# ryansynk/fastmax-experiments

Hardware: AMD Instinct MI355X
Metric: fastmax attn tokens/sec + achieved HBM GB/s at N=4096 d=64, 1/8 GPU (higher is better)
Workload: dtype f32; 1 GPU; fastmax p=1 masked fwd, (B,H,N,D)=(16,32,4096,64) per GPU, q,k,v~N(0,1) seed=rank, f32 I/O, fp32 accumulate; B_per_gpu=16, H=32, N=4096, D=64, global_batch=16, parallelism=dp1 (batch sharded, no data-path collective)

## Files before the change

fastmax_experiments_amd/csrc/fastmax_api.hip:

```cpp
#include "fastmax_common.h"

#include <climits>
#include <cstdlib>
#include <cstring>

using namespace fastmax;

namespace {
bool use_bf16_kernel(const fastmax_problem& p) {
    return mfma_bf16_supported(p) && tune_get(TUNE_BF16_KERNEL) != 0;
}
int validate(const fastmax_problem* p) {
    if (!p) return FASTMAX_E_NULL;
    if (p->p != 1 && p->p != 2) return FASTMAX_E_BAD_P;
    if (p->B <= 0 || p->H <= 0 || p->Nq <= 0 || p->Nk <= 0 || p->D <= 0 || p->D > FASTMAX_MAX_D)
        return FASTMAX_E_BAD_SHAPE;
    if (p->causal && p->Nq != p->Nk) return FASTMAX_E_BAD_SHAPE;
    if ((int64_t)p->B * p->H > 65535) return FASTMAX_E_BAD_SHAPE;
    if (p->in_dtype < 0 || p->in_dtype > 2 || p->out_dtype < 0 || p->out_dtype > 2) return FASTMAX_E_BAD_DTYPE;
    return FASTMAX_OK;
}
Strides3 st(const int64_t* s) { return Strides3{s[0], s[1], s[2]}; }

int select(const fastmax_problem& p) {
// ... 92 lines not shown
    if (p.path != FASTMAX_PATH_QUADRATIC_MFMA && has(lay, LAY_O)) {
        if (unmasked_lin_bwd_supported(p)) return FASTMAX_BWD_UNMASKED_LIN;
        if (lin_bwd_supported(p) && p.in_dtype == p.out_dtype) return FASTMAX_BWD_LIN;
        if (scan_bwd_supported(p)) return FASTMAX_BWD_SCAN;
    }
    return quad32_bwd_supported(p) ? FASTMAX_BWD_QUAD32 : FASTMAX_BWD_QUAD_MFMA;
}

int normalize_check(bool have_ptrs, int B, int H, int rep, int N, int D, const void* workspace, size_t workspace_bytes, size_t need,
                    int dtype = FASTMAX_F32) {
    if (!have_ptrs) return FASTMAX_E_NULL;
    if (B <= 0 || H <= 0 || rep <= 0 || N <= 0 || D <= 0 || D > FASTMAX_MAX_D) return FASTMAX_E_BAD_SHAPE;
    if (dtype < 0 || dtype > FASTMAX_F16) return FASTMAX_E_BAD_DTYPE;
    if (!workspace || workspace_bytes < need) return FASTMAX_E_WORKSPACE;
    return FASTMAX_OK;
}
}

namespace fastmax {
static bool mfma_variant_ok(int v) {
#ifdef FASTMAX_ABLATIONS
    if (v == 201 || (v >= 204 && v <= 209)) return true;
#endif
    return v == 200;
}
namespace {
struct TuneEntry { const char* name; const char* env; int value; };
TuneEntry g_tune[TUNE_COUNT] = {
    {"mfma_variant", "FASTMAX_MFMA_VARIANT", 200},
    {"bf16_kernel", "FASTMAX_BF16_KERNEL", 1},
    {"gemm_sched", "FASTMAX_GEMM_SCHED", 0},
    {"gemm_group_m", "FASTMAX_GEMM_GROUP_M", 16},
    {"gemm_xcd", "FASTMAX_GEMM_XCD", 1},
};
bool g_tune_loaded = false;
void tune_load() {
    if (g_tune_loaded) return;
    for (int i = 0; i < TUNE_COUNT; ++i) {
        const char* e = getenv(g_tune[i].env);
        if (!e) continue;
        if (i == TUNE_BF16_KERNEL) g_tune[i].value = e[0] == 'g' ? 0 : 1;
        else g_tune[i].value = atoi(e);
        if (i == TUNE_MFMA_VARIANT && !mfma_variant_ok(g_tune[i].value)) g_tune[i].value = 200;
    }
    g_tune_loaded = true;
}
}
int tune_get(int key) {
    tune_load();
    return g_tune[key].value;
}
int tune_set(const char* name, int value) {
    tune_load();
    for (int i = 0; i < TUNE_COUNT; ++i)
        if (!strcmp(name, g_tune[i].name)) {
            if (i == TUNE_MFMA_VARIANT && !mfma_variant_ok(value)) return FASTMAX_E_BAD_SHAPE;
            g_tune[i].value = value;
            return FASTMAX_OK;
        }
    return FASTMAX_E_BAD_SHAPE;
}
int tune_get_by_name(const char* name) {
    tune_load();
    for (int i = 0; i < TUNE_COUNT; ++i)
        if (!strcmp(name, g_tune[i].name)) return g_tune[i].value;
    return INT_MIN;
// ... 313 lines not shown
```

fastmax_experiments_amd/csrc/fastmax_common.h:

```cpp
#pragma once
#include <hip/hip_runtime.h>
#include <hip/hip_bf16.h>
#include <hip/hip_fp16.h>
#include <stdint.h>

#include "../../include/fastmax_hip.h"

namespace fastmax {

struct bf16_t { uint16_t bits; };
struct f16_t { _Float16 v; };

__device__ __forceinline__ float to_float(float x) { return x; }
__device__ __forceinline__ float to_float(bf16_t x) { return __uint_as_float(((uint32_t)x.bits) << 16); }
__device__ __forceinline__ float to_float(f16_t x) { return (float)x.v; }

__device__ __forceinline__ uint16_t f32_to_bf16_bits(float f) {
    __hip_bfloat16 h = __float2bfloat16(f);
    return *reinterpret_cast<uint16_t*>(&h);
}
template <typename T> __device__ __forceinline__ T from_float(float f);
template <> __device__ __forceinline__ float from_float<float>(float f) { return f; }
template <> __device__ __forceinline__ bf16_t from_float<bf16_t>(float f) { return bf16_t{f32_to_bf16_bits(f)}; }
template <> __device__ __forceinline__ f16_t from_float<f16_t>(float f) { return f16_t{(_Float16)f}; }
// ... 55 lines not shown
    int *nstar_q = nullptr, *nstar_k = nullptr;
};
struct FwdArgs {
    fastmax_problem prob;
    const void *q, *k, *v;
    Strides3 qs, ks, vs;
    void* o;
    float* g;
    void* workspace;
    size_t workspace_bytes;
    hipStream_t stream;
    const LinearmaxStats* stats = nullptr;
};
struct BwdArgs {
    fastmax_problem prob;
    const void *q, *k, *v, *o, *grad_o;
    const float* g;
    Strides3 qs, ks, vs, gos;
    void *dq, *dk, *dv;
    void* workspace;
    size_t workspace_bytes;
    hipStream_t stream;
    const float* fwd_states = nullptr;
    const float *qscale = nullptr, *kscale = nullptr;
    int fuse_prologue = 0;
    const int* k_nstar = nullptr;
    const int* q_nstar = nullptr;
};

int launch_fwd_quadratic(const FwdArgs& a);
int launch_fwd_recurrent_p1(const FwdArgs& a);
int launch_fwd_mfma_p1(const FwdArgs& a);
bool mfma_p1_supported(const fastmax_problem& p);
enum TuneKey { TUNE_MFMA_VARIANT = 0, TUNE_BF16_KERNEL = 1, TUNE_GEMM_SCHED = 2, TUNE_GEMM_GROUP_M = 3, TUNE_GEMM_XCD = 4, TUNE_COUNT };
int tune_get(int key);
int tune_set(const char* name, int value);
int tune_get_by_name(const char* name);
int launch_fwd_mfma_gen(const FwdArgs& a, const float* qscale, const float* kscale);
int launch_fwd_mfma_bf16(const FwdArgs& a, const float* qscale, const float* kscale);
bool mfma_bf16_supported(const fastmax_problem& p);
bool mfma_gen_supported(const fastmax_problem& p, bool norm);
int launch_normalize_cast(const void* x, Strides3 xs, int dtype, void* y, const float* inv_norm, int B, int H, int N, int D,
                          hipStream_t stream, const unsigned int* partials = nullptr, int npart = 0, float* inv_out = nullptr, int rep = 1);
int launch_normalize_partial_max(const void* x, Strides3 xs, int dtype, unsigned int* partials, int B, int H, int N, int D,
                                 hipStream_t stream);
size_t normalize_backward_workspace(int B, int H, int N);
size_t normalize_backward_workspace_grouped(int B, int G, int rep, int N);
int normalize_block_tokens(int rep);
int launch_normalize_backward(const void* x, Strides3 xs, int dtype, const void* gy, const float* inv_norm, void* gx, int B, int H,
                              int N, int D, void* ws, hipStream_t stream, int rep = 1);
int launch_normalize_stats(const void* x, Strides3 xs, int dtype, float* inv_norm, int B, int H, int N, int D,
                           void* workspace, hipStream_t stream);
int launch_normalize_stats2(const void* x0, Strides3 s0, const void* x1, Strides3 s1, int dtype, float* inv0, float* inv1, int B, int H,
                            int N, int D, void* ws, hipStream_t stream, int* nstar0 = nullptr, int* nstar1 = nullptr);
struct SplitPlan { int nseg, cps; };
SplitPlan split_plan(const fastmax_problem& p);
size_t split_workspace_bytes(const fastmax_problem& p, int dp);
int launch_split_states(const FwdArgs& a, const SplitPlan& plan, int dp, const float* kscale);
int linearmax_stats_and_states(const FwdArgs& a, const SplitPlan& plan, int dp);
bool unmasked_lin_supported(const fastmax_problem& p);
size_t unmasked_lin_workspace(const fastmax_problem& p);
int launch_fwd_unmasked_p1(const FwdArgs& a);
int launch_bwd_unmasked_p1(const BwdArgs& a);
size_t unmasked_lin_bwd_workspace(const fastmax_problem& p);
bool unmasked_lin_bwd_supported(const fastmax_problem& p);
int launch_bwd_prep_c(const BwdArgs& a, float* cbuf);
int launch_normalize_fixadd(const void* x, Strides3 xs, int dtype, const float* inv_norm, const float* part_dot,
// ... 29 lines not shown
```

fastmax_experiments_amd/csrc/fastmax_mfma32_common.h:

```cpp
#pragma once
#include "fastmax_mfma_common.h"

namespace fastmax {

typedef float f32x16 __attribute__((ext_vector_type(16)));

__device__ __forceinline__ f32x16 mfma32(const bf16x8 a, const bf16x8 b, f32x16 c) {
    return __builtin_amdgcn_mfma_f32_32x32x16_bf16(a, b, c, 0, 0, 0);
}
__device__ __forceinline__ f32x16 mfma32_c1(const bf16x8 a, const bf16x8 b) {
    f32x16 d;
    asm("s_nop 1\n\tv_mfma_f32_32x32x16_bf16 %0, %1, %2, 1.0\n\ts_nop 11" : "=&v"(d) : "v"(a), "v"(b));
    return d;
}
template <int NA, int NB>
__device__ __forceinline__ f32x16 mfma32_parts_c1(const Frag<NA>& a, const Frag<NB>& b) {
    f32x16 c = mfma32_c1(a.p[0], b.p[0]);
    if constexpr (NA == 2) c = mfma32(a.p[1], b.p[0], c);
    if constexpr (NB == 2) c = mfma32(a.p[0], b.p[1], c);
    return c;
}
template <int NA, int NB>
__device__ __forceinline__ f32x16 mfma32_parts(const Frag<NA>& a, const Frag<NB>& b, f32x16 c) {
    c = mfma32(a.p[0], b.p[0], c);
    if constexpr (NA == 2) c = mfma32(a.p[1], b.p[0], c);
    if constexpr (NB == 2) c = mfma32(a.p[0], b.p[1], c);
    return c;
}

__device__ __forceinline__ void mfma32_acc(f32x16& acc, const bf16x8 a, const bf16x8 b) {
    asm("s_nop 1\n\tv_mfma_f32_32x32x16_bf16 %0, %1, %2, %0" : "+a"(acc) : "v"(a), "v"(b));
}
template <int NA, int NB>
__device__ __forceinline__ void mfma32_parts_acc(f32x16& acc, const Frag<NA>& a, const Frag<NB>& b) {
    mfma32_acc(acc, a.p[0], b.p[0]);
    if constexpr (NA == 2) mfma32_acc(acc, a.p[1], b.p[0]);
    if constexpr (NB == 2) mfma32_acc(acc, a.p[0], b.p[1]);
}
// ... 118 lines not shown
```

fastmax_experiments_amd/csrc/fastmax_quad32_bwd.hip:

```cpp
#include "fastmax_mfma32_common.h"

#include <cmath>
#include <cstdlib>
#include <type_traits>

namespace fastmax {

struct Quad32BwdParams {
    const void *q, *k, *v, *gt;
    const float* cw;
    Strides3 qs, ks, vs;
    void *dq, *dk, *dv;
    int H, BH, Nq, Nk, D, causal, grad_dtype, nblk;
    float a;
};

__device__ __forceinline__ void quad32_block(int L, int nblk, int BH, int& bh, int& blk) {
    if ((BH & 7) == 0) {
        const int x = L & 7, m = L >> 3;
        bh = x + 8 * (m / nblk);
        blk = m % nblk;
    } else {
        bh = L / nblk;
        blk = L % nblk;
    }
}

template <int NPP> __device__ __forceinline__ void pack_tile(const float (&x)[16], Frag<NPP> (&f)[2]) {
#pragma unroll
    for (int s = 0; s < 2; ++s) {
        const f32x4 x0 = {x[8 * s], x[8 * s + 1], x[8 * s + 2], x[8 * s + 3]};
        const f32x4 x1 = {x[8 * s + 4], x[8 * s + 5], x[8 * s + 6], x[8 * s + 7]};
        if constexpr (NPP == 2) {
            bf16x4 h0, l0, h1, l1;
            split4(x0, h0, l0);
            split4(x1, h1, l1);
            f[s].p[0] = cat4(h0, h1);
            f[s].p[1] = cat4(l0, l1);
        } else {
            f[s].p[0] = cat4(to_bf16x4(x0), to_bf16x4(x1));
        }
    }
}

template <int NP, bool UNIT>
__device__ __forceinline__ f32x16 s_chain_head(const Frag<NP>& a, const Frag<NP>& b, const f32x16& cinit) {
    if constexpr (UNIT) return mfma32_parts_c1<NP, NP>(a, b);
    else return mfma32_parts<NP, NP>(a, b, cinit);
}

template <int DP, int P, typename TIN, int NW, int MB, bool UNIT>
__global__ __launch_bounds__(64 * NW, MB) void bwd32_dq_kernel(Quad32BwdParams prm) {
    constexpr int NP = InTraits<TIN>::NP, EPL = InTraits<TIN>::EPL, NPP = NP;
    constexpr int NT = 64 * NW, QT = 32 * NW;
    constexpr bool DUAL = DP == 128 && NP == 1;
    constexpr int SWR = DUAL ? 1 : 3, SWT = DUAL ? 2 : 3;
    constexpr int IMG = img_bytes<DP, SWR>(), IMGT = DUAL ? img_bytes<DP, SWT>() : 0;
    constexpr int KTO = 2 * NP * IMG, STAGE = 2 * NP * IMG + NP * IMGT;
    constexpr int COLS = DP / EPL, RPP = NT / COLS, NPASS = 64 / RPP;
    static_assert(RPP <= 64 && NPASS >= 1, "staging map");
    constexpr int KS = DP / 16, DT = DP / 32;
    constexpr bool ACC_A = DP == 128 && MB == 1;
    extern __shared__ __attribute__((aligned(16))) char smem[];
    const int tid = threadIdx.x, lane = tid & 63;
    const int w = __builtin_amdgcn_readfirstlane(tid >> 6);
    const int l31 = lane & 31, h = lane >> 5;
    int bh, qt;
    quad32_block(blockIdx.x, prm.nblk, prm.BH, bh, qt);
    const bool causal = prm.causal != 0;
    if (causal) qt = prm.nblk - 1 - qt;
    const int b = bh / prm.H, hh = bh % prm.H;
    const int D = prm.D, Nq = prm.Nq, Nk = prm.Nk;
    const int i0 = qt * QT, qw0 = i0 + 32 * w, myq = qw0 + l31;
    const TIN* qb = reinterpret_cast<const TIN*>(prm.q) + (int64_t)b * prm.qs.sb + (int64_t)hh * prm.qs.sh;
    const TIN* kb = reinterpret_cast<const TIN*>(prm.k) + (int64_t)b * prm.ks.sb + (int64_t)hh * prm.ks.sh;
    const TIN* vb = reinterpret_cast<const TIN*>(prm.v) + (int64_t)b * prm.vs.sb + (int64_t)hh * prm.vs.sh;
    const TIN* gb = reinterpret_cast<const TIN*>(prm.gt) + (int64_t)bh * Nq * D;
    const int srow = tid / COLS, scol = tid % COLS;

    Frag<NP> qf[KS], gf[KS];
#pragma unroll
    for (int ks = 0; ks < KS; ++ks) {
        if constexpr (P == 2) {
            if constexpr (UNIT) qf[ks] = load_q_frag_scaled<TIN>(qb, prm.qs.sn, myq, Nq, 16 * ks + 8 * h, D, prm.a);
            else qf[ks] = load_q_frag<TIN>(qb, prm.qs.sn, myq, Nq, 16 * ks + 8 * h, D);
        }
        gf[ks] = load_q_frag<TIN>(gb, D, myq, Nq, 16 * ks + 8 * h, D);
    }
    const int qc = myq < Nq ? myq : Nq - 1;
    const float ncw = -prm.cw[(int64_t)bh * Nq + qc];
    f32x16 ucinit, scinit;
#pragma unroll
    for (int i = 0; i < 16; ++i) { ucinit[i] = ncw; scinit[i] = 1.0f / prm.a; }
    const int klim = causal ? min(myq, Nk - 1) : Nk - 1;

    u32x4 rk[NPASS], rv[NPASS];
    const TileKernelLoader<TIN, NPASS, RPP> kload(kb, prm.ks.sn, Nk, D, srow, scol), vload(vb, prm.vs.sn, Nk, D, srow, scol);
    auto request = [&](int kt) __attribute__((always_inline)) {
        kload.load(kt, rk);
        vload.load(kt, rv);
    };
// ... 87 lines not shown
        advance(kt);
        tile(kt, kt & 1, std::true_type{});
        __syncthreads();
    }
    for (; kt < nkt; ++kt) {
        advance(kt);
        __syncthreads();
    }
    if constexpr (ACC_A) {
#pragma unroll
        for (int mt = 0; mt < DT; ++mt) acc_fence(acc[mt]);
    }
    const float oscale = (P == 2 && !UNIT) ? prm.a * prm.a : prm.a;
    store_tile32_t<DT>(smem + w * 4096, acc, oscale, lane, prm.dq, prm.grad_dtype, (int64_t)bh * Nq, qw0, Nq, D);
}

template <int DP, int P, typename TIN, int NW, bool UNIT>
__global__ __launch_bounds__(64 * NW, (DP == 64 && InTraits<TIN>::NP == 1 && NW == 4) ? 2 : 1) void bwd32_dkv_kernel(Quad32BwdParams prm) {
    constexpr int NP = InTraits<TIN>::NP, EPL = InTraits<TIN>::EPL, NPP = NP;
    constexpr int NT = 64 * NW, KT = 32 * NW;
    constexpr bool DUAL = DP == 128 && NP == 1;
    constexpr int SWR = DUAL ? 1 : 3, SWT = DUAL ? 2 : 3;
    constexpr int IMG = img_bytes<DP, SWR>(), IMGT = DUAL ? img_bytes<DP, SWT>() : 0;
    constexpr int TRO = 2 * NP * IMG, CWO = TRO + 2 * NP * IMGT, STAGE = CWO + 256;
    constexpr int COLS = DP / EPL, RPP = NT / COLS, NPASS = 64 / RPP;
    static_assert(RPP <= 64 && NPASS >= 1, "staging map");
    constexpr int KS = DP / 16, DT = DP / 32;
    constexpr bool ACC_A = DP == 128 && NW == 4;
    extern __shared__ __attribute__((aligned(16))) char smem[];
    const int tid = threadIdx.x, lane = tid & 63;
    const int w = __builtin_amdgcn_readfirstlane(tid >> 6);
    const int l31 = lane & 31, h = lane >> 5;
    int bh, kb_;
    quad32_block(blockIdx.x, prm.nblk, prm.BH, bh, kb_);
    const bool causal = prm.causal != 0;
    const int b = bh / prm.H, hh = bh % prm.H;
    const int D = prm.D, Nq = prm.Nq, Nk = prm.Nk;
    const int j0 = kb_ * KT, jw0 = j0 + 32 * w, myk = jw0 + l31;
    const TIN* qb = reinterpret_cast<const TIN*>(prm.q) + (int64_t)b * prm.qs.sb + (int64_t)hh * prm.qs.sh;
    const TIN* kb = reinterpret_cast<const TIN*>(prm.k) + (int64_t)b * prm.ks.sb + (int64_t)hh * prm.ks.sh;
    const TIN* vb = reinterpret_cast<const TIN*>(prm.v) + (int64_t)b * prm.vs.sb + (int64_t)hh * prm.vs.sh;
    const TIN* gb = reinterpret_cast<const TIN*>(prm.gt) + (int64_t)bh * Nq * D;
    const int srow = tid / COLS, scol = tid % COLS;

    Frag<NP> kf[KS], vf[KS];
#pragma unroll
    for (int ks = 0; ks < KS; ++ks) {
        if constexpr (UNIT) kf[ks] = load_q_frag_scaled<TIN>(kb, prm.ks.sn, myk, Nk, 16 * ks + 8 * h, D, prm.a);
        else kf[ks] = load_q_frag<TIN>(kb, prm.ks.sn, myk, Nk, 16 * ks + 8 * h, D);
        vf[ks] = load_q_frag<TIN>(vb, prm.vs.sn, myk, Nk, 16 * ks + 8 * h, D);
    }
    const float u0 = UNIT ? 1.0f : 1.0f / prm.a, c0 = u0 * u0;
    f32x16 scinit;
#pragma unroll
    for (int i = 0; i < 16; ++i) scinit[i] = u0;
    const int qlo = myk < Nk ? (causal ? myk : 0) : 0x7fffffff;

    u32x4 rq[NPASS], rg[NPASS];
    float rcw = 0.f;
    const TileKernelLoader<TIN, NPASS, RPP> qload(qb, prm.qs.sn, Nq, D, srow, scol), gload(gb, D, Nq, D, srow, scol);
    auto request = [&](int it) __attribute__((always_inline)) {
        qload.load(it, rq);
        gload.load(it, rg);
        if (tid < 64) {
            const int gi = it * 64 + tid, gc = gi < Nq ? gi : Nq - 1;
            rcw = prm.cw[(int64_t)bh * Nq + gc];
        }
// ... 245 lines not shown
    for (; it < it_q; ++it) {
        advance(it);
        tile(it, (it - it0) & 1, std::false_type{});
        __syncthreads();
    }
    for (; it < nqt; ++it) {
        advance(it);
        tile(it, (it - it0) & 1, std::true_type{});
        __syncthreads();
    }
    if constexpr (ACC_A) {
#pragma unroll
        for (int t = 0; t < DT; ++t) { acc_fence(dkacc[t]); acc_fence(dvacc[t]); }
    }
    const float e1 = (P == 2 && !UNIT) ? prm.a : 1.0f;
    const float e2 = (P == 1 ? 1.0f : 0.5f) * (UNIT ? 1.0f : (P == 1 ? prm.a : prm.a * prm.a));
    store_tile32_t<DT>(smem + w * 4096, dkacc, prm.a * e1, lane, prm.dk, prm.grad_dtype, (int64_t)bh * Nk, jw0, Nk, D);
    store_tile32_t<DT>(smem + w * 4096, dvacc, e2, lane, prm.dv, prm.grad_dtype, (int64_t)bh * Nk, jw0, Nk, D);
}

template <int DP, int P, typename TIN, int NW, int MB, bool UNIT>
static int launch_bwd32_dq(Quad32BwdParams prm, hipStream_t stream) {
    constexpr int NP = InTraits<TIN>::NP;
    constexpr int st_q = 2 * ((DP == 128 && NP == 1) ? NP * (2 * img_bytes<DP, 1>() + img_bytes<DP, 2>()) : 2 * NP * img_bytes<DP, 3>()), epi = NW * 4096;
    constexpr int lds_q = st_q > epi ? st_q : epi;
    auto kq = bwd32_dq_kernel<DP, P, TIN, NW, MB, UNIT>;
    static bool attr_set = false;
    if (!attr_set) {
        hipError_t e = hipFuncSetAttribute(reinterpret_cast<const void*>(kq), hipFuncAttributeMaxDynamicSharedMemorySize, lds_q);
        if (e != hipSuccess) return (int)e;
        attr_set = true;
    }
    prm.nblk = (prm.Nq + 32 * NW - 1) / (32 * NW);
    hipLaunchKernelGGL(kq, dim3(prm.nblk * prm.BH), dim3(64 * NW), lds_q, stream, prm);
    return (int)hipGetLastError();
}
template <int DP, int P, typename TIN, int NW, bool UNIT>
static int launch_bwd32_dkv(Quad32BwdParams prm, hipStream_t stream) {
    constexpr int NP = InTraits<TIN>::NP;
    constexpr int st_kv = 2 * (((DP == 128 && NP == 1) ? 2 * NP * (img_bytes<DP, 1>() + img_bytes<DP, 2>()) : 2 * NP * img_bytes<DP, 3>()) + 256), epi = NW * 4096;
    constexpr int lds_kv = st_kv > epi ? st_kv : epi;
    auto kkv = bwd32_dkv_kernel<DP, P, TIN, NW, UNIT>;
    static bool attr_set = false;
    if (!attr_set) {
        hipError_t e = hipFuncSetAttribute(reinterpret_cast<const void*>(kkv), hipFuncAttributeMaxDynamicSharedMemorySize, lds_kv);
        if (e != hipSuccess) return (int)e;
        attr_set = true;
    }
    prm.nblk = (prm.Nk + 32 * NW - 1) / (32 * NW);
    hipLaunchKernelGGL(kkv, dim3(prm.nblk * prm.BH), dim3(64 * NW), lds_kv, stream, prm);
    return (int)hipGetLastError();
}
template <int DP, int P, typename TIN, bool UNIT>
static int launch_bwd32_n(const Quad32BwdParams& prm, hipStream_t stream) {
    constexpr int NP = InTraits<TIN>::NP;
    int rc;
    if constexpr (DP == 64 && NP == 2) rc = launch_bwd32_dq<DP, P, TIN, 8, 1, UNIT>(prm, stream);
    else if constexpr (DP == 64) rc = launch_bwd32_dq<DP, P, TIN, 4, 2, UNIT>(prm, stream);
    else rc = launch_bwd32_dq<DP, P, TIN, 4, 1, UNIT>(prm, stream);
    if (rc) return rc;
    if constexpr (DP == 64 && NP == 2) return launch_bwd32_dkv<DP, P, TIN, 8, UNIT>(prm, stream);
    else return launch_bwd32_dkv<DP, P, TIN, 4, UNIT>(prm, stream);
}
static bool is_pow2(float a) { int e; return a > 0.f && frexpf(a, &e) == 0.5f; }
template <int DP, int P, typename TIN>
static int launch_bwd32_u(const Quad32BwdParams& prm, hipStream_t stream) {
    if constexpr (InTraits<TIN>::NP == 2) return launch_bwd32_n<DP, P, TIN, true>(prm, stream);
    else return is_pow2(prm.a) ? launch_bwd32_n<DP, P, TIN, true>(prm, stream) : launch_bwd32_n<DP, P, TIN, false>(prm, stream);
}
template <int P, typename TIN>
static int launch_bwd32_d(const Quad32BwdParams& prm, hipStream_t stream) {
    return prm.D <= 64 ? launch_bwd32_u<64, P, TIN>(prm, stream) : launch_bwd32_u<128, P, TIN>(prm, stream);
}
template <typename TIN>
static int launch_bwd32_p(const Quad32BwdParams& prm, int p, hipStream_t stream) {
    return p == 1 ? launch_bwd32_d<1, TIN>(prm, stream) : launch_bwd32_d<2, TIN>(prm, stream);
}

bool quad32_bwd_supported(const fastmax_problem& p) {
    static const int mode = [] { const char* e = getenv("FASTMAX_QUAD32_BWD"); return e ? atoi(e) : 1; }();
    if (!mode) return false;
    const int epl = p.in_dtype == FASTMAX_F32 ? 4 : 8;
// ... 23 lines not shown
```

fastmax_experiments_amd/csrc/fastmax_quad32_mfma.hip:

```cpp
#include "fastmax_mfma32_common.h"

#include <cmath>
#include <cstdlib>
#include <type_traits>

namespace fastmax {

struct Quad32Params {
    const void *q, *k, *v;
    Strides3 qs, ks, vs;
    void* o;
    float* g;
    int H, BH, Nq, Nk, D, causal, out_dtype, nqt;
    float a, g0;
};

template <int DP, typename TIN, int NPP, int NW, int QB> constexpr int quad32_min_blocks() {
    if (QB == 2) return 2;
    if (DP == 64 && InTraits<TIN>::NP == 1 && NPP == 1) return NW == 8 ? 1 : 3;
    return NW == 8 ? 1 : 2;
}

template <int DP, int P, typename TIN, int NPP, int NW, bool UNIT, int SCHED, int QB>
__global__ __launch_bounds__(64 * NW, (quad32_min_blocks<DP, TIN, NPP, NW, QB>())) void fwd_quad32_kernel(Quad32Params prm) {
    constexpr int NP = InTraits<TIN>::NP, EPL = InTraits<TIN>::EPL;
    constexpr int NT = 64 * NW, QW = 32 * QB, QT = QW * NW;
    constexpr int KIMG = img_bytes<DP, 1>(), VIMG = img_bytes<DP, 2>(), STAGE = NP * (KIMG + VIMG);
    constexpr int COLS = DP / EPL, RPP = NT / COLS, NPASS = 64 / RPP;
    static_assert(RPP <= 64 && NPASS >= 1, "staging map");
    static_assert(QB == 1 || (NP == 1 && NPP == 1), "two query blocks per wave: single-part operands only");
    constexpr int KS = DP / 16, DT = DP / 32;
    extern __shared__ __attribute__((aligned(16))) char smem[];
    const int tid = threadIdx.x, lane = tid & 63;
    const int w = __builtin_amdgcn_readfirstlane(tid >> 6);
    const int l31 = lane & 31, h = lane >> 5;
    int bh, qt;
    {
        const int L = blockIdx.x, nqt = prm.nqt;
        if ((prm.BH & 7) == 0) {
            const int x = L & 7, m = L >> 3;
            bh = x + 8 * (m / nqt);
            qt = m % nqt;
        } else {
            bh = L / nqt;
            qt = L % nqt;
        }
        if (prm.causal) qt = nqt - 1 - qt;
    }
    const int b = bh / prm.H, hh = bh % prm.H;
    const int D = prm.D, Nq = prm.Nq, Nk = prm.Nk;
    const bool causal = prm.causal != 0;
    const int i0 = qt * QT, qw0 = i0 + QW * w;
    const TIN* qb = reinterpret_cast<const TIN*>(prm.q) + (int64_t)b * prm.qs.sb + (int64_t)hh * prm.qs.sh;
    const TIN* kb = reinterpret_cast<const TIN*>(prm.k) + (int64_t)b * prm.ks.sb + (int64_t)hh * prm.ks.sh;
    const TIN* vb = reinterpret_cast<const TIN*>(prm.v) + (int64_t)b * prm.vs.sb + (int64_t)hh * prm.vs.sh;
    const int srow = tid / COLS, scol = tid % COLS;

    Frag<NP> qf[QB][KS];
    int klim[QB];
#pragma unroll
    for (int qb_ = 0; qb_ < QB; ++qb_) {
        const int myq = qw0 + 32 * qb_ + l31;
        klim[qb_] = causal ? min(myq, Nk - 1) : Nk - 1;
#pragma unroll
        for (int ks = 0; ks < KS; ++ks) {
            if constexpr (UNIT) qf[qb_][ks] = load_q_frag_scaled<TIN>(qb, prm.qs.sn, myq, Nq, 16 * ks + 8 * h, D, prm.a);
            else qf[qb_][ks] = load_q_frag<TIN>(qb, prm.qs.sn, myq, Nq, 16 * ks + 8 * h, D);
        }
    }

    u32x4 rk[NPASS], rv[NPASS];
    const TileKernelLoader<TIN, NPASS, RPP> kload(kb, prm.ks.sn, Nk, D, srow, scol), vload(vb, prm.vs.sn, Nk, D, srow, scol);
    auto request = [&](int kt) __attribute__((always_inline)) {
        kload.load(kt, rk);
        vload.load(kt, rv);
    };
    auto commit = [&](int stage) __attribute__((always_inline)) {
#pragma unroll
        for (int ps = 0; ps < NPASS; ++ps) {
            stage_piece<DP, TIN, 1>(smem, stage * STAGE, srow + ps * RPP, scol, rk[ps]);
            stage_piece<DP, TIN, 2>(smem, stage * STAGE + NP * KIMG, srow + ps * RPP, scol, rv[ps]);
        }
    };
    const int nkt = causal ? min((i0 + QT + 63) / 64, (Nk + 63) / 64) : (Nk + 63) / 64;

    f32x16 oacc[QB][DT];
    float gsum[QB][4];
#pragma unroll
    for (int qb_ = 0; qb_ < QB; ++qb_) {
#pragma unroll
        for (int dt = 0; dt < DT; ++dt)
#pragma unroll
            for (int i = 0; i < 16; ++i) oacc[qb_][dt][i] = 0.f;
#pragma unroll
        for (int i = 0; i < 4; ++i) gsum[qb_][i] = 0.f;
    }
    const float u0 = UNIT ? 1.0f : 1.0f / prm.a, c0 = u0 * u0;
    const float fscale = (P == 1 ? 1.0f : 0.5f) * (UNIT ? 1.0f : (P == 1 ? prm.a : prm.a * prm.a));
    f32x16 cinit;
#pragma unroll
    for (int i = 0; i < 16; ++i) cinit[i] = u0;

    auto poly = [&](const f32x16& sc, int qb_, int key0, auto masked_tag, Frag<NPP> (&pf)[2]) {
        constexpr bool MASKED = decltype(masked_tag)::value;
        float pv[16];
        const int rel = klim[qb_] - key0 - 4 * h;
#pragma unroll
        for (int i = 0; i < 16; ++i) {
            float x = sc[i];
            if constexpr (P == 2) x = fmaf(x, x, c0);
            if constexpr (MASKED) x = ((i & 3) + 8 * (i >> 2) <= rel) ? x : 0.f;
            pv[i] = x;
            gsum[qb_][i & 3] += x;
        }
#pragma unroll
        for (int s = 0; s < 2; ++s) {
            const f32x4 x0 = {pv[8 * s], pv[8 * s + 1], pv[8 * s + 2], pv[8 * s + 3]};
            const f32x4 x1 = {pv[8 * s + 4], pv[8 * s + 5], pv[8 * s + 6], pv[8 * s + 7]};
            if constexpr (NPP == 2) {
                bf16x4 h0, l0, h1, l1;
                split4(x0, h0, l0);
                split4(x1, h1, l1);
                pf[s].p[0] = cat4(h0, h1);
                pf[s].p[1] = cat4(l0, l1);
            } else {
                pf[s].p[0] = cat4(to_bf16x4(x0), to_bf16x4(x1));
            }
        }
    };
    auto qk_chain = [&](const Frag<NP> (&kf)[KS], int qb_) {
        f32x16 sc;
        if constexpr (UNIT) sc = mfma32_parts_c1<NP, NP>(kf[0], qf[qb_][0]);
        else sc = mfma32_parts<NP, NP>(kf[0], qf[qb_][0], cinit);
#pragma unroll
        for (int ks = 1; ks < KS; ++ks) sc = mfma32_parts<NP, NP>(kf[ks], qf[qb_][ks], sc);
        return sc;
    };
    constexpr int QKM = KS * (NP == 2 ? 3 : 1);
    constexpr int PVM = 2 * DT * (1 + (NP == 2) + (NPP == 2));

    auto tile1 = [&](int kt, int stage, auto masked_tag) __attribute__((always_inline)) {
        constexpr bool MASKED = decltype(masked_tag)::value;
        constexpr int VPOLY = (P == 2 ? 16 : 0) + 16 + (NPP == 2 ? 40 : 8) + (MASKED ? 32 : 0);
        const int KI = stage * STAGE, VI = KI + NP * KIMG, k0 = kt * 64;
        f32x16 sc[2];
        Frag<NP> kf[2][KS];
#pragma unroll
        for (int jt = 0; jt < 2; ++jt)
#pragma unroll
            for (int ks = 0; ks < KS; ++ks)
#pragma unroll
                for (int p = 0; p < NP; ++p) kf[jt][ks].p[p] = ld_row8<DP, 1>(smem, KI + p * KIMG, 32 * jt + l31, 2 * ks + h);
        Frag<NP> vf[2][2][DT];
        auto vread = [&](int jt) __attribute__((always_inline)) {
#pragma unroll
            for (int s = 0; s < 2; ++s)
#pragma unroll
                for (int dt = 0; dt < DT; ++dt)
#pragma unroll
                    for (int p = 0; p < NP; ++p) vf[jt][s][dt].p[p] = ld_tr8_32<DP>(smem, VI + p * VIMG, 32 * jt + 16 * s, 32 * dt, lane);
        };
        Frag<NPP> pf[2][2];
        auto pv = [&](int jt) __attribute__((always_inline)) {
#pragma unroll
            for (int s = 0; s < 2; ++s)
#pragma unroll
                for (int dt = 0; dt < DT; ++dt) oacc[0][dt] = mfma32_parts<NP, NPP>(vf[jt][s][dt], pf[jt][s], oacc[0][dt]);
        };
        if constexpr (SCHED == 1) {
            sc[0] = qk_chain(kf[0], 0);
            vread(0);
            __builtin_amdgcn_sched_barrier(0);
            sc[1] = qk_chain(kf[1], 0);
            poly(sc[0], 0, k0, masked_tag, pf[0]);
#pragma unroll
            for (int i = 0; i < QKM; ++i) {
                __builtin_amdgcn_sched_group_barrier(0x008, 1, 0);
                __builtin_amdgcn_sched_group_barrier(0x002, (VPOLY + QKM - 1) / QKM, 0);
            }
            __builtin_amdgcn_sched_barrier(0);
            vread(1);
            pv(0);
            poly(sc[1], 0, k0 + 32, masked_tag, pf[1]);
#pragma unroll
            for (int i = 0; i < PVM; ++i) {
                __builtin_amdgcn_sched_group_barrier(0x008, 1, 1);
                __builtin_amdgcn_sched_group_barrier(0x002, (VPOLY + PVM - 1) / PVM, 1);
            }
            __builtin_amdgcn_sched_barrier(0);
            pv(1);
        } else {
            sc[0] = qk_chain(kf[0], 0);
            sc[1] = qk_chain(kf[1], 0);
#pragma unroll
            for (int jt = 0; jt < 2; ++jt) {
                vread(jt);
                __builtin_amdgcn_sched_barrier(0);
                poly(sc[jt], 0, k0 + 32 * jt, masked_tag, pf[jt]);
                __builtin_amdgcn_sched_barrier(0);
                pv(jt);
            }
        }
    };

    auto tile2 = [&](int kt, int stage, auto masked_tag) __attribute__((always_inline)) {
        constexpr bool MASKED = decltype(masked_tag)::value;
        constexpr int VPOLY = (P == 2 ? 16 : 0) + 16 + 8 + (MASKED ? 32 : 0);
        const int KI = stage * STAGE, VI = KI + NP * KIMG, k0 = kt * 64;
        constexpr int B1 = QB - 1;
        auto kread = [&](int jt, Frag<NP> (&kf)[KS]) {
#pragma unroll
            for (int ks = 0; ks < KS; ++ks) kf[ks].p[0] = ld_row8<DP, 1>(smem, KI, 32 * jt + l31, 2 * ks + h);
        };
        auto vread = [&](int jt, Frag<NP> (&vf)[2][DT]) {
#pragma unroll
            for (int s = 0; s < 2; ++s)
#pragma unroll
                for (int dt = 0; dt < DT; ++dt) vf[s][dt].p[0] = ld_tr8_32<DP>(smem, VI, 32 * jt + 16 * s, 32 * dt, lane);
        };
        auto pv = [&](int qb_, const Frag<NP> (&vf)[2][DT], const Frag<NPP> (&pf)[2]) {
#pragma unroll
            for (int s = 0; s < 2; ++s)
#pragma unroll
                for (int dt = 0; dt < DT; ++dt) oacc[qb_][dt] = mfma32_parts<NP, NPP>(vf[s][dt], pf[s], oacc[qb_][dt]);
        };
        auto group = [&](auto id_tag) __attribute__((always_inline)) {
            constexpr int ID = decltype(id_tag)::value;
            if constexpr (SCHED == 1) {
#pragma unroll
                for (int i = 0; i < 4; ++i) {
                    __builtin_amdgcn_sched_group_barrier(0x008, 1, ID);
// ... 1 lines not shown
                }
            }
        };
        Frag<NP> kf0[KS], kf1[KS], vf0[2][DT], vf1[2][DT];
        Frag<NPP> pa0[2], pb0[2], pa1[2], pb1[2];
        kread(0, kf0);
        kread(1, kf1);
        f32x16 sa0 = qk_chain(kf0, 0);
        f32x16 sb0 = qk_chain(kf0, B1);
        vread(0, vf0);
        __builtin_amdgcn_sched_barrier(0);
        f32x16 sa1 = qk_chain(kf1, 0);
        poly(sa0, 0, k0, masked_tag, pa0);
        group(std::integral_constant<int, 0>{});
        __builtin_amdgcn_sched_barrier(0);
        f32x16 sb1 = qk_chain(kf1, B1);
        poly(sb0, B1, k0, masked_tag, pb0);
        group(std::integral_constant<int, 1>{});
        __builtin_amdgcn_sched_barrier(0);
        vread(1, vf1);
        pv(0, vf0, pa0);
        poly(sa1, 0, k0 + 32, masked_tag, pa1);
        group(std::integral_constant<int, 2>{});
        __builtin_amdgcn_sched_barrier(0);
        pv(B1, vf0, pb0);
        poly(sb1, B1, k0 + 32, masked_tag, pb1);
        group(std::integral_constant<int, 3>{});
        __builtin_amdgcn_sched_barrier(0);
        pv(0, vf1, pa1);
        pv(B1, vf1, pb1);
    };
    auto tile = [&](int kt, int stage, auto masked_tag) __attribute__((always_inline)) {
        if constexpr (QB == 2) tile2(kt, stage, masked_tag);
        else tile1(kt, stage, masked_tag);
    };
    auto advance = [&](int kt) __attribute__((always_inline)) {
        if (kt + 1 < nkt) {
            commit((kt & 1) ^ 1);
            if (kt + 2 < nkt) request(kt + 2);
        }
    };
    const int n_full = Nk / 64;
    const int n_plain = causal ? min((qw0 + 1) / 64, n_full) : n_full;
    const int n_act = causal ? min(nkt, (qw0 + QW - 1) / 64 + 1) : nkt;

    request(0);
    commit(0);
    if (nkt > 1) request(1);
    __syncthreads();
    int kt = 0;
    for (; kt < n_plain; ++kt) {
        advance(kt);
        tile(kt, kt & 1, std::false_type{});
        __syncthreads();
    }
    for (; kt < n_act; ++kt) {
        advance(kt);
        tile(kt, kt & 1, std::true_type{});
        __syncthreads();
    }
    for (; kt < nkt; ++kt) {
        advance(kt);
        __syncthreads();
    }

#pragma unroll
    for (int qb_ = 0; qb_ < QB; ++qb_) {
        const int myq = qw0 + 32 * qb_ + l31;
        float gs = (gsum[qb_][0] + gsum[qb_][1]) + (gsum[qb_][2] + gsum[qb_][3]);
        gs += __shfl_xor(gs, 32, 64);
        gs *= fscale;
        const float gval = causal ? gs : gs - (float)Nk + prm.g0;
        if (myq < Nq && prm.g && h == 0) prm.g[(int64_t)bh * Nq + myq] = gval;
        const float ginv = fscale / gval;
        store_tile32_t<DT>(smem + w * 4096, oacc[qb_], ginv, lane, prm.o, prm.out_dtype, (int64_t)bh * Nq, qw0 + 32 * qb_, Nq, D);
    }
}

template <int DP, int P, typename TIN, int NPP, int NW, bool UNIT, int SCHED, int QB>
static int launch_quad32_w(Quad32Params prm, hipStream_t stream) {
    constexpr int NP = InTraits<TIN>::NP;
    constexpr int stages = 2 * NP * (img_bytes<DP, 1>() + img_bytes<DP, 2>()), epi = NW * 4096;
    constexpr int lds = stages > epi ? stages : epi;
    auto kern = fwd_quad32_kernel<DP, P, TIN, NPP, NW, UNIT, SCHED, QB>;
    static bool attr_set = false;
    if (!attr_set) {
        hipError_t e = hipFuncSetAttribute(reinterpret_cast<const void*>(kern), hipFuncAttributeMaxDynamicSharedMemorySize, lds);
        if (e != hipSuccess) return (int)e;
        attr_set = true;
    }
    prm.nqt = (prm.Nq + 32 * QB * NW - 1) / (32 * QB * NW);
    hipLaunchKernelGGL(kern, dim3(prm.nqt * prm.BH), dim3(64 * NW), lds, stream, prm);
    return (int)hipGetLastError();
}
template <int DP, int P, typename TIN, int NPP, bool UNIT>
static int launch_quad32_n(const Quad32Params& prm, hipStream_t stream) {
    if constexpr (InTraits<TIN>::NP == 1 && NPP == 1 && DP == 64) {
        if (prm.Nq >= 1024) return launch_quad32_w<DP, P, TIN, NPP, 4, UNIT, 1, 2>(prm, stream);
        return launch_quad32_w<DP, P, TIN, NPP, 4, UNIT, 0, 1>(prm, stream);
    } else {
        constexpr int NWD = (DP == 64 && InTraits<TIN>::NP == 1) ? 4 : 8;
        return launch_quad32_w<DP, P, TIN, NPP, NWD, UNIT, DP == 128 ? 1 : 0, 1>(prm, stream);
    }
}
static bool is_pow2(float a) { int e; return a > 0.f && frexpf(a, &e) == 0.5f; }
template <int DP, int P, typename TIN, int NPP>
static int launch_quad32_u(const Quad32Params& prm, hipStream_t stream) {
    if constexpr (InTraits<TIN>::NP == 2) return launch_quad32_n<DP, P, TIN, NPP, true>(prm, stream);
    else return is_pow2(prm.a) ? launch_quad32_n<DP, P, TIN, NPP, true>(prm, stream) : launch_quad32_n<DP, P, TIN, NPP, false>(prm, stream);
}
template <int DP, int P, typename TIN>
static int launch_quad32_t(const Quad32Params& prm, hipStream_t stream) {
    if constexpr (InTraits<TIN>::NP == 1) {
        if (prm.out_dtype != FASTMAX_F32) return launch_quad32_u<DP, P, TIN, 1>(prm, stream);
    }
    return launch_quad32_u<DP, P, TIN, 2>(prm, stream);
}
template <int P, typename TIN>
static int launch_quad32_d(const Quad32Params& prm, hipStream_t stream) {
    if constexpr (InTraits<TIN>::NP == 2) {
        return prm.D <= 64 ? launch_quad32_t<64, P, TIN>(prm, stream) : FASTMAX_E_BAD_SHAPE;
    } else {
        return prm.D <= 64 ? launch_quad32_t<64, P, TIN>(prm, stream) : launch_quad32_t<128, P, TIN>(prm, stream);
    }
// ... 30 lines not shown
```

Baseline: 162.7 million tokens/s.

## Balance causal quad32 work by folding query rows and grouping heads per block

For causal attention with two query sub-blocks per warp, each warp now pairs a low query tile with its mirrored high tile, so every block does roughly equal work across the triangular mask. For other configurations, block-to-head mapping groups G heads together so concurrently scheduled blocks span mixed causal lengths while sharing L2-resident K/V. This targets tail imbalance from causal blocks of very different lengths. It adds mapping arithmetic and a second per-sub-block tile loop, and it changes the order in which K/V are reused.

```diff
diff --git a/fastmax_experiments_amd/csrc/fastmax_api.hip b/fastmax_experiments_amd/csrc/fastmax_api.hip
--- a/fastmax_experiments_amd/csrc/fastmax_api.hip
+++ b/fastmax_experiments_amd/csrc/fastmax_api.hip
@@ -148,6 +148,7 @@
     {"gemm_sched", "FASTMAX_GEMM_SCHED", 0},
     {"gemm_group_m", "FASTMAX_GEMM_GROUP_M", 16},
     {"gemm_xcd", "FASTMAX_GEMM_XCD", 1},
+    {"p2_balance", "FASTMAX_P2_BALANCE", 1},
 };
 bool g_tune_loaded = false;
 void tune_load() {
diff --git a/fastmax_experiments_amd/csrc/fastmax_common.h b/fastmax_experiments_amd/csrc/fastmax_common.h
--- a/fastmax_experiments_amd/csrc/fastmax_common.h
+++ b/fastmax_experiments_amd/csrc/fastmax_common.h
@@ -111,7 +111,7 @@
 int launch_fwd_recurrent_p1(const FwdArgs& a);
 int launch_fwd_mfma_p1(const FwdArgs& a);
 bool mfma_p1_supported(const fastmax_problem& p);
-enum TuneKey { TUNE_MFMA_VARIANT = 0, TUNE_BF16_KERNEL = 1, TUNE_GEMM_SCHED = 2, TUNE_GEMM_GROUP_M = 3, TUNE_GEMM_XCD = 4, TUNE_COUNT };
+enum TuneKey { TUNE_MFMA_VARIANT = 0, TUNE_BF16_KERNEL = 1, TUNE_GEMM_SCHED = 2, TUNE_GEMM_GROUP_M = 3, TUNE_GEMM_XCD = 4, TUNE_P2_BALANCE = 5, TUNE_COUNT };
 int tune_get(int key);
 int tune_set(const char* name, int value);
 int tune_get_by_name(const char* name);
diff --git a/fastmax_experiments_amd/csrc/fastmax_mfma32_common.h b/fastmax_experiments_amd/csrc/fastmax_mfma32_common.h
--- a/fastmax_experiments_amd/csrc/fastmax_mfma32_common.h
+++ b/fastmax_experiments_amd/csrc/fastmax_mfma32_common.h
@@ -4,6 +4,25 @@
 namespace fastmax {
 
 typedef float f32x16 __attribute__((ext_vector_type(16)));
+
+__device__ __forceinline__ void quad32_block(int L, int nblk, int BH, int G, int& bh, int& blk) {
+    const bool xcd = (BH & 7) == 0;
+    const int m = xcd ? L >> 3 : L, heads = xcd ? BH >> 3 : BH;
+    const int grp = m / (G * nblk), r = m - grp * G * nblk;
+    const int gh = min(G, heads - grp * G);
+    const int hl = grp * G + r % gh;
+    blk = r / gh;
+    bh = xcd ? (L & 7) + 8 * hl : hl;
+}
+inline int quad32_group_heads(int causal, int slots, int nblk, int64_t head_bytes) {
+    const int mode = tune_get(TUNE_P2_BALANCE);
+    if (!causal || mode <= 0) return 1;
+    if (mode > 1) return mode;
+    const int64_t cover = (slots + nblk - 1) / nblk, want = cover > 4 ? cover : 4;
+    const int64_t cap = (8 << 20) / (head_bytes > 0 ? head_bytes : 1);
+    const int64_t g = want < cap ? want : cap;
+    return g < 1 ? 1 : (int)g;
+}
 
 __device__ __forceinline__ f32x16 mfma32(const bf16x8 a, const bf16x8 b, f32x16 c) {
     return __builtin_amdgcn_mfma_f32_32x32x16_bf16(a, b, c, 0, 0, 0);
diff --git a/fastmax_experiments_amd/csrc/fastmax_quad32_bwd.hip b/fastmax_experiments_amd/csrc/fastmax_quad32_bwd.hip
--- a/fastmax_experiments_amd/csrc/fastmax_quad32_bwd.hip
+++ b/fastmax_experiments_amd/csrc/fastmax_quad32_bwd.hip
@@ -13,18 +13,8 @@
     void *dq, *dk, *dv;
     int H, BH, Nq, Nk, D, causal, grad_dtype, nblk;
     float a;
+    int G;
 };
-
-__device__ __forceinline__ void quad32_block(int L, int nblk, int BH, int& bh, int& blk) {
-    if ((BH & 7) == 0) {
-        const int x = L & 7, m = L >> 3;
-        bh = x + 8 * (m / nblk);
-        blk = m % nblk;
-    } else {
-        bh = L / nblk;
-        blk = L % nblk;
-    }
-}
 
 template <int NPP> __device__ __forceinline__ void pack_tile(const float (&x)[16], Frag<NPP> (&f)[2]) {
 #pragma unroll
@@ -66,7 +56,7 @@
     const int w = __builtin_amdgcn_readfirstlane(tid >> 6);
     const int l31 = lane & 31, h = lane >> 5;
     int bh, qt;
-    quad32_block(blockIdx.x, prm.nblk, prm.BH, bh, qt);
+    quad32_block(blockIdx.x, prm.nblk, prm.BH, prm.G, bh, qt);
     const bool causal = prm.causal != 0;
     if (causal) qt = prm.nblk - 1 - qt;
     const int b = bh / prm.H, hh = bh % prm.H;
@@ -220,7 +210,7 @@
     const int w = __builtin_amdgcn_readfirstlane(tid >> 6);
     const int l31 = lane & 31, h = lane >> 5;
     int bh, kb_;
-    quad32_block(blockIdx.x, prm.nblk, prm.BH, bh, kb_);
+    quad32_block(blockIdx.x, prm.nblk, prm.BH, prm.G, bh, kb_);
     const bool causal = prm.causal != 0;
     const int b = bh / prm.H, hh = bh % prm.H;
     const int D = prm.D, Nq = prm.Nq, Nk = prm.Nk;
@@ -532,6 +522,7 @@
         attr_set = true;
     }
     prm.nblk = (prm.Nq + 32 * NW - 1) / (32 * NW);
+    prm.G = quad32_group_heads(prm.causal, 32 * MB, prm.nblk, 2 * (int64_t)prm.Nk * DP * sizeof(TIN));
     hipLaunchKernelGGL(kq, dim3(prm.nblk * prm.BH), dim3(64 * NW), lds_q, stream, prm);
     return (int)hipGetLastError();
 }
@@ -548,6 +539,8 @@
         attr_set = true;
     }
     prm.nblk = (prm.Nk + 32 * NW - 1) / (32 * NW);
+    constexpr int WPC = (DP == 64 && NW == 4) ? 2 : 1;
+    prm.G = quad32_group_heads(prm.causal, 32 * WPC, prm.nblk, 2 * (int64_t)prm.Nq * DP * sizeof(TIN));
     hipLaunchKernelGGL(kkv, dim3(prm.nblk * prm.BH), dim3(64 * NW), lds_kv, stream, prm);
     return (int)hipGetLastError();
 }
diff --git a/fastmax_experiments_amd/csrc/fastmax_quad32_mfma.hip b/fastmax_experiments_amd/csrc/fastmax_quad32_mfma.hip
--- a/fastmax_experiments_amd/csrc/fastmax_quad32_mfma.hip
+++ b/fastmax_experiments_amd/csrc/fastmax_quad32_mfma.hip
@@ -13,6 +13,7 @@
     float* g;
     int H, BH, Nq, Nk, D, causal, out_dtype, nqt;
     float a, g0;
+    int G, fold;
 };
 
 template <int DP, typename TIN, int NPP, int NW, int QB> constexpr int quad32_min_blocks() {
@@ -35,22 +36,20 @@
     const int w = __builtin_amdgcn_readfirstlane(tid >> 6);
     const int l31 = lane & 31, h = lane >> 5;
     int bh, qt;
-    {
-        const int L = blockIdx.x, nqt = prm.nqt;
-        if ((prm.BH & 7) == 0) {
-            const int x = L & 7, m = L >> 3;
-            bh = x + 8 * (m / nqt);
-            qt = m % nqt;
-        } else {
-            bh = L / nqt;
-            qt = L % nqt;
-        }
-        if (prm.causal) qt = nqt - 1 - qt;
-    }
+    quad32_block(blockIdx.x, prm.nqt, prm.BH, prm.G, bh, qt);
+    if (prm.causal) qt = prm.nqt - 1 - qt;
     const int b = bh / prm.H, hh = bh % prm.H;
     const int D = prm.D, Nq = prm.Nq, Nk = prm.Nk;
     const bool causal = prm.causal != 0;
-    const int i0 = qt * QT, qw0 = i0 + QW * w;
+    const int i0 = qt * QT;
+    const bool fold = QB == 2 && prm.fold;
+    int r0[QB];
+#pragma unroll
+    for (int qb_ = 0; qb_ < QB; ++qb_) r0[qb_] = i0 + QW * w + 32 * qb_;
+    if (fold) {
+        r0[0] = 32 * (4 * qt + w);
+        r0[QB - 1] = 32 * (8 * prm.nqt - 1 - (4 * qt + w));
+    }
     const TIN* qb = reinterpret_cast<const TIN*>(prm.q) + (int64_t)b * prm.qs.sb + (int64_t)hh * prm.qs.sh;
     const TIN* kb = reinterpret_cast<const TIN*>(prm.k) + (int64_t)b * prm.ks.sb + (int64_t)hh * prm.ks.sh;
     const TIN* vb = reinterpret_cast<const TIN*>(prm.v) + (int64_t)b * prm.vs.sb + (int64_t)hh * prm.vs.sh;
@@ -60,7 +59,7 @@
     int klim[QB];
 #pragma unroll
     for (int qb_ = 0; qb_ < QB; ++qb_) {
-        const int myq = qw0 + 32 * qb_ + l31;
+        const int myq = r0[qb_] + l31;
         klim[qb_] = causal ? min(myq, Nk - 1) : Nk - 1;
 #pragma unroll
         for (int ks = 0; ks < KS; ++ks) {
@@ -82,7 +81,12 @@
             stage_piece<DP, TIN, 2>(smem, stage * STAGE + NP * KIMG, srow + ps * RPP, scol, rv[ps]);
         }
     };
-    const int nkt = causal ? min((i0 + QT + 63) / 64, (Nk + 63) / 64) : (Nk + 63) / 64;
+    int iend = i0 + QT;
+    if (fold) {
+        const int nbq = (Nq + 31) / 32, top = 8 * prm.nqt - 4 * qt;
+        iend = 32 * (top - 4 >= nbq ? 4 * qt + 4 : min(top, nbq));
+    }
+    const int nkt = causal ? min((iend + 63) / 64, (Nk + 63) / 64) : (Nk + 63) / 64;
 
     f32x16 oacc[QB][DT];
     float gsum[QB][4];
@@ -139,8 +143,9 @@
     constexpr int QKM = KS * (NP == 2 ? 3 : 1);
     constexpr int PVM = 2 * DT * (1 + (NP == 2) + (NPP == 2));
 
-    auto tile1 = [&](int kt, int stage, auto masked_tag) __attribute__((always_inline)) {
+    auto tile1 = [&](int kt, int stage, auto blk_tag, auto masked_tag) __attribute__((always_inline)) {
         constexpr bool MASKED = decltype(masked_tag)::value;
+        constexpr int QI = decltype(blk_tag)::value;
         constexpr int VPOLY = (P == 2 ? 16 : 0) + 16 + (NPP == 2 ? 40 : 8) + (MASKED ? 32 : 0);
         const int KI = stage * STAGE, VI = KI + NP * KIMG, k0 = kt * 64;
         f32x16 sc[2];
@@ -165,14 +170,14 @@
 #pragma unroll
             for (int s = 0; s < 2; ++s)
 #pragma unroll
-                for (int dt = 0; dt < DT; ++dt) oacc[0][dt] = mfma32_parts<NP, NPP>(vf[jt][s][dt], pf[jt][s], oacc[0][dt]);
+                for (int dt = 0; dt < DT; ++dt) oacc[QI][dt] = mfma32_parts<NP, NPP>(vf[jt][s][dt], pf[jt][s], oacc[QI][dt]);
         };
         if constexpr (SCHED == 1) {
-            sc[0] = qk_chain(kf[0], 0);
+            sc[0] = qk_chain(kf[0], QI);
             vread(0);
             __builtin_amdgcn_sched_barrier(0);
-            sc[1] = qk_chain(kf[1], 0);
-            poly(sc[0], 0, k0, masked_tag, pf[0]);
+            sc[1] = qk_chain(kf[1], QI);
+            poly(sc[0], QI, k0, masked_tag, pf[0]);
 #pragma unroll
             for (int i = 0; i < QKM; ++i) {
                 __builtin_amdgcn_sched_group_barrier(0x008, 1, 0);
@@ -181,7 +186,7 @@
             __builtin_amdgcn_sched_barrier(0);
             vread(1);
             pv(0);
-            poly(sc[1], 0, k0 + 32, masked_tag, pf[1]);
+            poly(sc[1], QI, k0 + 32, masked_tag, pf[1]);
 #pragma unroll
             for (int i = 0; i < PVM; ++i) {
                 __builtin_amdgcn_sched_group_barrier(0x008, 1, 1);
@@ -190,13 +195,13 @@
             __builtin_amdgcn_sched_barrier(0);
             pv(1);
         } else {
-            sc[0] = qk_chain(kf[0], 0);
-            sc[1] = qk_chain(kf[1], 0);
+            sc[0] = qk_chain(kf[0], QI);
+            sc[1] = qk_chain(kf[1], QI);
 #pragma unroll
             for (int jt = 0; jt < 2; ++jt) {
                 vread(jt);
                 __builtin_amdgcn_sched_barrier(0);
-                poly(sc[jt], 0, k0 + 32 * jt, masked_tag, pf[jt]);
+                poly(sc[jt], QI, k0 + 32 * jt, masked_tag, pf[jt]);
                 __builtin_amdgcn_sched_barrier(0);
                 pv(jt);
             }
@@ -264,7 +269,10 @@
     };
     auto tile = [&](int kt, int stage, auto masked_tag) __attribute__((always_inline)) {
         if constexpr (QB == 2) tile2(kt, stage, masked_tag);
-        else tile1(kt, stage, masked_tag);
+        else tile1(kt, stage, std::integral_constant<int, 0>{}, masked_tag);
+    };
+    auto tile_last = [&](int kt, int stage, auto masked_tag) __attribute__((always_inline)) {
+        tile1(kt, stage, std::integral_constant<int, QB - 1>{}, masked_tag);
     };
     auto advance = [&](int kt) __attribute__((always_inline)) {
         if (kt + 1 < nkt) {
@@ -273,24 +281,41 @@
         }
     };
     const int n_full = Nk / 64;
-    const int n_plain = causal ? min((qw0 + 1) / 64, n_full) : n_full;
-    const int n_act = causal ? min(nkt, (qw0 + QW - 1) / 64 + 1) : nkt;
+    int n_plain[QB], n_act[QB];
+#pragma unroll
+    for (int qb_ = 0; qb_ < QB; ++qb_) {
+        const int r = (qb_ > 0 && r0[qb_] >= Nq) ? r0[0] : r0[qb_];
+        n_plain[qb_] = causal ? min((r + 1) / 64, n_full) : n_full;
+        n_act[qb_] = causal ? min(nkt, (r + 31) / 64 + 1) : nkt;
+    }
 
     request(0);
     commit(0);
     if (nkt > 1) request(1);
     __syncthreads();
     int kt = 0;
-    for (; kt < n_plain; ++kt) {
+    for (; kt < n_plain[0]; ++kt) {
         advance(kt);
         tile(kt, kt & 1, std::false_type{});
         __syncthreads();
     }
-    for (; kt < n_act; ++kt) {
+    for (; kt < n_act[0]; ++kt) {
         advance(kt);
         tile(kt, kt & 1, std::true_type{});
         __syncthreads();
     }
+    if constexpr (QB == 2) {
+        for (; kt < n_plain[1]; ++kt) {
+            advance(kt);
+            tile_last(kt, kt & 1, std::false_type{});
+            __syncthreads();
+        }
+        for (; kt < n_act[1]; ++kt) {
+            advance(kt);
+            tile_last(kt, kt & 1, std::true_type{});
+            __syncthreads();
+        }
+    }
     for (; kt < nkt; ++kt) {
         advance(kt);
         __syncthreads();
@@ -298,14 +323,14 @@
 
 #pragma unroll
     for (int qb_ = 0; qb_ < QB; ++qb_) {
-        const int myq = qw0 + 32 * qb_ + l31;
+        const int myq = r0[qb_] + l31;
         float gs = (gsum[qb_][0] + gsum[qb_][1]) + (gsum[qb_][2] + gsum[qb_][3]);
         gs += __shfl_xor(gs, 32, 64);
         gs *= fscale;
         const float gval = causal ? gs : gs - (float)Nk + prm.g0;
         if (myq < Nq && prm.g && h == 0) prm.g[(int64_t)bh * Nq + myq] = gval;
         const float ginv = fscale / gval;
-        store_tile32_t<DT>(smem + w * 4096, oacc[qb_], ginv, lane, prm.o, prm.out_dtype, (int64_t)bh * Nq, qw0 + 32 * qb_, Nq, D);
+        store_tile32_t<DT>(smem + w * 4096, oacc[qb_], ginv, lane, prm.o, prm.out_dtype, (int64_t)bh * Nq, r0[qb_], Nq, D);
     }
 }
 
@@ -322,6 +347,9 @@
         attr_set = true;
     }
     prm.nqt = (prm.Nq + 32 * QB * NW - 1) / (32 * QB * NW);
+    prm.fold = QB == 2 && prm.causal && tune_get(TUNE_P2_BALANCE) > 0;
+    prm.G = QB == 2 ? 1 : quad32_group_heads(prm.causal, 32 * quad32_min_blocks<DP, TIN, NPP, NW, QB>(), prm.nqt,
+                                             2 * (int64_t)prm.Nk * DP * sizeof(TIN));
     hipLaunchKernelGGL(kern, dim3(prm.nqt * prm.BH), dim3(64 * NW), lds, stream, prm);
     return (int)hipGetLastError();
 }
```

Result: no change. 162.9 million tokens/s (median of 2 runs) (+0.1%).
